# hzi-bifo/RiboDetector

Measured on AMD Instinct MI355X. Metric: reads/sec classified, 100 bp paired-end, higher is better.
Workload: dtype f16x3-split (f32 accumulate); 1 GPU; BASELINE configs[2]: paired-end 100 bp, --ensure rrna, 1048576 pairs/step/GPU x 47 steps (49.3 M total); pinned host bytes -> H2D -> kernels -> labels D2H (SURVEY 8d region ii); read_len=100, ensure=rrna, kernel_variant=mfma_f16x3_t32, parallelism=reads sharded x1, label gather to rank 0, rccl_ranks=1, forced_dist=False, prefix_k=12

## Files before the change

ribodetector_amd/csrc/rd_fastq_index.hpp:

```cpp
#pragma once
#include "rd_common.hpp"

namespace {

constexpr int FQ_THREADS = 256;
constexpr int FQ_BYTES = 64;
constexpr int FQ_TILE = FQ_THREADS * FQ_BYTES;

struct FqSummary {
    int64_t begin, end, n_lines, n_records, consumed;
    unsigned long long bad_record;
    int32_t status, dirty;
    int64_t reserved;
};
static_assert(sizeof(FqSummary) == 64 && sizeof(rd_fq_summary) == 64, "rd_fq_summary layout");

__device__ __forceinline__ bool fq_is_ws(unsigned c) {
    return c == ' ' || (c >= 9 && c <= 13) || (c >= 0x1c && c <= 0x1f) || c == 0x85 || c == 0xa0;
}

__device__ __forceinline__ uint64_t fq_newline_mask(const uint8_t *__restrict__ text, int64_t o, int64_t begin, int64_t end) {
    if (o >= end || o + FQ_BYTES <= begin) return 0;
    const u32x4 *p = reinterpret_cast<const u32x4 *>(text + o);
    uint64_t m = 0;
#pragma unroll
    for (int q = 0; q < 4; ++q) {
        const u32x4 v = p[q];
#pragma unroll
        for (int k = 0; k < 4; ++k) {
            const uint32_t x = v[k] ^ 0x0a0a0a0au;
            const uint32_t z = ~(((x & 0x7f7f7f7fu) + 0x7f7f7f7fu) | x | 0x7f7f7f7fu);
            const uint64_t nib = (((z >> 7) * 0x204081u) >> 21) & 0xfu;
            m |= nib << (16 * q + 4 * k);
        }
    }
    const int lo = begin > o ? (int)(begin - o) : 0, hi = end - o < FQ_BYTES ? (int)(end - o) : FQ_BYTES;
    if (lo > 0) m &= ~0ull << lo;
    if (hi < 64) m &= ~(~0ull << hi);
    return m;
}

__device__ __forceinline__ uint32_t fq_block_scan(uint32_t v, uint32_t *sh, uint32_t &total) {
    const int tid = threadIdx.x, lane = tid & 63, wave = tid >> 6;
    uint32_t inc = v;
#pragma unroll
    for (int o = 1; o < 64; o <<= 1) {
        const uint32_t t = __shfl_up(inc, o);
        if (lane >= o) inc += t;
    }
    if (lane == 63) sh[wave] = inc;
    __syncthreads();
    uint32_t base = 0;
    for (int w = 0; w < wave; ++w) base += sh[w];
    total = sh[0] + sh[1] + sh[2] + sh[3];
    __syncthreads();
    return base + inc - v;
}

template <bool TEXT>
__global__ __launch_bounds__(FQ_THREADS) void rd_fq_begin_kernel(uint8_t *__restrict__ text, int64_t pad, int64_t end, const uint8_t *__restrict__ prev_text,
                                                                const FqSummary *__restrict__ prev, int final, FqSummary *__restrict__ sum) {
    __shared__ int64_t s_begin;
    __shared__ int s_status;
    if (threadIdx.x == 0) {
        int64_t begin = pad;
        int status = RD_FQ_OK;
        if (prev) {
            const int64_t carry = prev->end - prev->consumed;
            if (prev->status != RD_FQ_OK) status = RD_FQ_CHAIN;
            else if (carry < 0 || carry > pad) status = RD_FQ_CARRY;
            else begin = pad - carry;
        }
        s_begin = begin;
        s_status = status;
    }
    __syncthreads();
    const int64_t begin = s_begin;
    if (prev && s_status == RD_FQ_OK) {
        const uint8_t *src = prev_text + prev->consumed;
        for (int64_t i = threadIdx.x; i < pad - begin; i += FQ_THREADS) text[begin + i] = src[i];
    }
    __syncthreads();
    if (threadIdx.x == 0) {
        int64_t e = end;
        if (TEXT && final && e > begin && text[e - 1] != '\n') text[e++] = '\n';
        sum->begin = begin;
        sum->end = e;
        sum->n_lines = sum->n_records = 0;
        sum->consumed = begin;
        sum->bad_record = ~0ull;
        sum->status = s_status;
        sum->dirty = 0;
        sum->reserved = 0;
    }
}

__global__ __launch_bounds__(FQ_THREADS) void rd_fq_count_kernel(const uint8_t *__restrict__ text, const FqSummary *__restrict__ sum,
                                                                uint32_t *__restrict__ tile_count) {
    __shared__ uint32_t sh[4];
    const int64_t o = (int64_t)blockIdx.x * FQ_TILE + (int64_t)threadIdx.x * FQ_BYTES;
    const uint64_t m = sum->status == RD_FQ_OK ? fq_newline_mask(text, o, sum->begin, sum->end) : 0;
    uint32_t total;
    fq_block_scan((uint32_t)__popcll(m), sh, total);
    if (threadIdx.x == 0) tile_count[blockIdx.x] = total;
}

__global__ __launch_bounds__(FQ_THREADS) void rd_fq_scan_kernel(uint32_t *__restrict__ tile_count, int ntiles, FqSummary *__restrict__ sum, int64_t cap_lines) {
    __shared__ uint32_t sh[4];
    __shared__ uint32_t run_s;
    if (threadIdx.x == 0) run_s = 0;
    __syncthreads();
    for (int b0 = 0; b0 < ntiles; b0 += FQ_THREADS) {
        const int b = b0 + threadIdx.x;
        const uint32_t v = b < ntiles ? tile_count[b] : 0;
        uint32_t total;
        const uint32_t ex = fq_block_scan(v, sh, total);
        const uint32_t run = run_s;
        if (b < ntiles) tile_count[b] = run + ex;
        __syncthreads();
        if (threadIdx.x == 0) run_s = run + total;
        __syncthreads();
    }
    if (threadIdx.x == 0) {
        int64_t lines = run_s;
        if (lines > cap_lines) {
            sum->status = RD_FQ_LINES;
            lines = 0;
        }
        sum->n_lines = lines;
        sum->n_records = lines / 4;
    }
}

__global__ __launch_bounds__(FQ_THREADS) void rd_fq_fill_kernel(const uint8_t *__restrict__ text, const FqSummary *__restrict__ sum,
                                                               const uint32_t *__restrict__ tile_base, int32_t *__restrict__ line_end) {
    __shared__ uint32_t sh[4];
    if (sum->status != RD_FQ_OK) return;
    const int64_t o = (int64_t)blockIdx.x * FQ_TILE + (int64_t)threadIdx.x * FQ_BYTES;
    uint64_t m = fq_newline_mask(text, o, sum->begin, sum->end);
    uint32_t total;
    uint32_t j = tile_base[blockIdx.x] + fq_block_scan((uint32_t)__popcll(m), sh, total);
    while (m) {
        const int b = __ffsll((long long)m) - 1;
        line_end[j++] = (int32_t)(o + b);
        m &= m - 1;
    }
}

__device__ __forceinline__ int64_t fq_line_start(const int32_t *__restrict__ line_end, int64_t j, int64_t begin) {
    return j ? (int64_t)line_end[j - 1] + 1 : begin;
}

__global__ __launch_bounds__(FQ_THREADS) void rd_fq_check_kernel(const uint8_t *__restrict__ text, const int32_t *__restrict__ line_end,
                                                                FqSummary *__restrict__ sum, int final) {
    if (sum->status != RD_FQ_OK && sum->status != RD_FQ_TRUNCATED) return;
    const int64_t n = sum->n_records, begin = sum->begin, L = sum->n_lines;
    const int64_t stride = (int64_t)gridDim.x * FQ_THREADS;
    bool dirty = false;
    for (int64_t r = (int64_t)blockIdx.x * FQ_THREADS + threadIdx.x; r < n; r += stride) {
        int64_t ls = fq_line_start(line_end, 4 * r, begin);
        if (text[ls] != '@') atomicMin(&sum->bad_record, (unsigned long long)r);
#pragma unroll
        for (int k = 0; k < 4; ++k) {
            const int64_t p = line_end[4 * r + k];
            dirty |= p > ls && fq_is_ws(text[p - 1]);
            ls = p + 1;
        }
    }
    if (dirty) sum->dirty = 1;
    if (blockIdx.x == 0 && threadIdx.x == 0) {
        int64_t consumed = n ? (int64_t)line_end[4 * n - 1] + 1 : begin;
        if (final) {
            bool trunc = false, ws = false;
            for (int64_t j = 4 * n; j < L; ++j) {
                const int64_t ls = fq_line_start(line_end, j, begin), p = line_end[j];
                if (p > ls) {
                    if (fq_is_ws(text[p - 1])) ws = true; else trunc = true;
                }
            }
            if (ws) sum->dirty = 1;
            else if (trunc) sum->status = RD_FQ_TRUNCATED;
            consumed = sum->end;
        }
        sum->consumed = consumed;
    }
}

__global__ void rd_fq_verdict_kernel(FqSummary *__restrict__ sum) {
    if ((sum->status == RD_FQ_OK || sum->status == RD_FQ_TRUNCATED) && sum->bad_record != ~0ull && !sum->dirty) sum->status = RD_FQ_HEADER;
}

__global__ __launch_bounds__(FQ_THREADS) void rd_fq_gather_kernel(const uint8_t *__restrict__ text, const int32_t *__restrict__ line_end,
                                                                 const FqSummary *__restrict__ sum, int64_t lo, int64_t hi,
                                                                 uint8_t *__restrict__ out_text, int64_t out_cap, const int64_t *__restrict__ cursor_in,
                                                                 int64_t *__restrict__ cursor_out, int64_t *__restrict__ rec_start,
                                                                 int64_t *__restrict__ seq_off, int32_t *__restrict__ seq_len) {
    const int64_t begin = sum->begin;
    const int64_t d0 = *cursor_in;
    const bool framed = sum->status == RD_FQ_OK || sum->status == RD_FQ_HEADER || sum->status == RD_FQ_TRUNCATED;
    const bool ok = framed && hi <= sum->n_records && lo <= hi && d0 >= 0;
    const int64_t src0 = ok ? fq_line_start(line_end, 4 * lo, begin) : 0, src1 = ok ? fq_line_start(line_end, 4 * hi, begin) : 0;
    const int64_t nbytes = src1 - src0;
    const int64_t gtid = (int64_t)blockIdx.x * FQ_THREADS + threadIdx.x, stride = (int64_t)gridDim.x * FQ_THREADS;
    if (!ok || d0 + nbytes > out_cap) {
        if (gtid == 0) *cursor_out = -1;
        return;
    }
    const uint8_t *src = text + src0;
    const int64_t d1 = d0 + nbytes;
    for (int64_t o = (d0 & ~(int64_t)15) + 16 * gtid; o < d1; o += 16 * stride) {
        const int64_t a = o < d0 ? d0 : o, e = o + 16 < d1 ? o + 16 : d1;
        if (a == o && e == o + 16) {
            u32x4 v;
            __builtin_memcpy(&v, src + (o - d0), 16);
            *reinterpret_cast<u32x4 *>(out_text + o) = v;
        } else {
            for (int64_t q = a; q < e; ++q) out_text[q] = src[q - d0];
        }
    }
    const int64_t shift = d0 - src0;
    for (int64_t i = gtid; i < hi - lo; i += stride) {
        const int64_t r = lo + i;
        const int64_t rs = fq_line_start(line_end, 4 * r, begin), so = (int64_t)line_end[4 * r] + 1;
        rec_start[i] = rs + shift;
        seq_off[i] = so + shift;
        seq_len[i] = (int32_t)((int64_t)line_end[4 * r + 1] - so);
    }
    if (gtid == 0) {
        rec_start[hi - lo] = d1;
        *cursor_out = d1;
    }
}

__global__ __launch_bounds__(FQ_THREADS) void rd_fq_strip_mark_kernel(const uint8_t *__restrict__ text, const int32_t *__restrict__ line_end,
                                                                     const FqSummary *__restrict__ sum, uint8_t *__restrict__ del) {
    const int64_t L = sum->n_lines, begin = sum->begin;
    const int64_t stride = (int64_t)gridDim.x * FQ_THREADS;
    for (int64_t j = (int64_t)blockIdx.x * FQ_THREADS + threadIdx.x; j < L; j += stride) {
        const int64_t ls = fq_line_start(line_end, j, begin);
        for (int64_t q = line_end[j]; q > ls && fq_is_ws(text[q - 1]); --q) del[q - 1] = 1;
    }
}

__global__ __launch_bounds__(FQ_THREADS) void rd_fq_sample_kernel(const int32_t *__restrict__ line_end, const FqSummary *__restrict__ sum, int64_t every,
                                                                 int32_t *__restrict__ samples, int64_t cap) {
    const bool framed = sum->status == RD_FQ_OK || sum->status == RD_FQ_HEADER || sum->status == RD_FQ_TRUNCATED;
    const int64_t n = framed ? sum->n_records : -1, begin = sum->begin;
    const int64_t stride = (int64_t)gridDim.x * FQ_THREADS;
    for (int64_t k = (int64_t)blockIdx.x * FQ_THREADS + threadIdx.x; k < cap; k += stride)
        samples[k] = k * every <= n ? (int32_t)fq_line_start(line_end, 4 * k * every, begin) : -1;
}

constexpr int COPY_THREADS = 1024;
__global__ __launch_bounds__(COPY_THREADS) void rd_copy_kernel(uint8_t *__restrict__ dst, const uint8_t *__restrict__ src, int64_t n) {
    const int64_t gtid = (int64_t)blockIdx.x * blockDim.x + threadIdx.x, stride = (int64_t)gridDim.x * blockDim.x;
    const int64_t head = (16 - ((uintptr_t)dst & 15)) & 15;
    if (gtid < head && gtid < n) dst[gtid] = src[gtid];
    const int64_t body = n > head ? (n - head) / 16 : 0;
    u32x4 *d = reinterpret_cast<u32x4 *>(dst + head);
    const uint8_t *s0 = src + head;
    int64_t i = gtid;
    for (; i + 3 * stride < body; i += 4 * stride) {
        u32x4 v0, v1, v2, v3;
        __builtin_memcpy(&v0, s0 + 16 * i, 16);
        __builtin_memcpy(&v1, s0 + 16 * (i + stride), 16);
        __builtin_memcpy(&v2, s0 + 16 * (i + 2 * stride), 16);
        __builtin_memcpy(&v3, s0 + 16 * (i + 3 * stride), 16);
        d[i] = v0; d[i + stride] = v1; d[i + 2 * stride] = v2; d[i + 3 * stride] = v3;
    }
    for (; i < body; i += stride) {
        u32x4 v;
        __builtin_memcpy(&v, s0 + 16 * i, 16);
        d[i] = v;
    }
    const int64_t tail0 = head + 16 * body;
    if (tail0 + gtid < n && gtid < 16) dst[tail0 + gtid] = src[tail0 + gtid];
}

struct FqWs {
    int ntiles;
    uint32_t *tiles;
    size_t total;
};
FqWs fq_ws(Carver &c, int64_t text_end) {
    FqWs p;
    p.ntiles = (int)((text_end + 1 + FQ_TILE - 1) / FQ_TILE);
    if (p.ntiles < 1) p.ntiles = 1;
    p.tiles = c.take<uint32_t>((size_t)p.ntiles);
    p.total = c.off;
    return p;
}
FqWs fq_ws(void *workspace, int64_t text_end) {
    Carver c(workspace);
    return fq_ws(c, text_end);
}

int fq_index_check(const char *fn, const uint8_t *text, int64_t pad, int64_t end, const uint8_t *prev_text, const rd_fq_summary *prev, const int32_t *line_end,
                   int64_t cap_lines, const rd_fq_summary *summary, const void *workspace, bool fa_null, bool fa_bad, const uint8_t *norm) {
    if (!text || !line_end || !summary || !workspace || fa_null) RD_FAIL(RD_E_INVALID, "%s: null pointer", fn);
    if (pad < 0 || end < pad || end >= 0x7fffffffLL - 64 || cap_lines < 0 || fa_bad)
        RD_FAIL(RD_E_INVALID, "%s: bad pad / end / cap_lines%s (a batch buffer is < 2 GiB)", fn, norm ? " / norm_cap / cap_records" : "");
    if ((prev == nullptr) != (prev_text == nullptr)) RD_FAIL(RD_E_INVALID, "%s: prev and prev_text go together", fn);
    if (((uintptr_t)text & 63) || ((uintptr_t)workspace & 255) || ((uintptr_t)norm & 15))
        RD_FAIL(RD_E_INVALID, "%s: text must be 64-byte aligned, workspace 256-byte aligned%s", fn, norm ? ", norm 16-byte aligned" : "");
    return RD_OK;
}

void fq_line_table(uint8_t *text, int64_t pad, int64_t end, const uint8_t *prev_text, const rd_fq_summary *prev, int32_t final, int32_t *line_end, int64_t cap_lines,
                   FqSummary *sum, const FqWs &w, hipStream_t st) {
    hipLaunchKernelGGL(rd_fq_begin_kernel<true>, dim3(1), dim3(FQ_THREADS), 0, st, text, pad, end, prev_text, (const FqSummary *)prev, (int)final, sum);
    hipLaunchKernelGGL(rd_fq_count_kernel, dim3(w.ntiles), dim3(FQ_THREADS), 0, st, text, sum, w.tiles);
    hipLaunchKernelGGL(rd_fq_scan_kernel, dim3(1), dim3(FQ_THREADS), 0, st, w.tiles, w.ntiles, sum, cap_lines);
    hipLaunchKernelGGL(rd_fq_fill_kernel, dim3(w.ntiles), dim3(FQ_THREADS), 0, st, text, sum, w.tiles, line_end);
}

template <typename K, typename... T>
int fq_gather(const char *fn, K kernel, const rd_fq_summary *summary, int64_t rec_lo, int64_t rec_hi, int64_t max_bytes, uint8_t *out_text, int64_t out_cap,
              const int64_t *cursor_in, int64_t *cursor_out, int64_t *rec_start, int64_t *seq_off, int32_t *seq_len, void *stream, T... tables) {
    if ((... || !tables) || !summary || !out_text || !cursor_in || !cursor_out || !rec_start || !seq_off || !seq_len) RD_FAIL(RD_E_INVALID, "%s: null pointer", fn);
    if (rec_lo < 0 || rec_hi < rec_lo || max_bytes < 0 || out_cap < 0 || cursor_in == cursor_out) RD_FAIL(RD_E_INVALID, "%s: bad range", fn);
    if ((uintptr_t)out_text & 15) RD_FAIL(RD_E_INVALID, "%s: out_text must be 16-byte aligned", fn);
    int64_t grid = max_bytes / (16 * FQ_THREADS * 4) + 1;
    const int64_t grid_r = (rec_hi - rec_lo) / FQ_THREADS + 1;
    if (grid < grid_r) grid = grid_r;
    if (grid > 8192) grid = 8192;
    hipLaunchKernelGGL(kernel, dim3((unsigned)grid), dim3(FQ_THREADS), 0, (hipStream_t)stream, tables..., (const FqSummary *)summary, rec_lo, rec_hi, out_text, out_cap,
                       cursor_in, cursor_out, rec_start, seq_off, seq_len);
    RD_HIP(hipGetLastError());
    return RD_OK;
}

template <typename K, typename T>
int fq_sample(const char *fn, K kernel, const T *table, const rd_fq_summary *summary, int64_t every, int32_t *samples, int64_t cap, void *stream) {
    if (!table || !summary || !samples || every < 1 || cap < 0) RD_FAIL(RD_E_INVALID, "%s: bad argument", fn);
    if (cap == 0) return RD_OK;
    int64_t grid = cap / FQ_THREADS + 1;
    if (grid > 1024) grid = 1024;
    hipLaunchKernelGGL(kernel, dim3((unsigned)grid), dim3(FQ_THREADS), 0, (hipStream_t)stream, table, (const FqSummary *)summary, every, samples, cap);
    RD_HIP(hipGetLastError());
    return RD_OK;
}

}
```

ribodetector_amd/csrc/rd_kernels.hip:

```cpp
#include <stdlib.h>
#include "rd_common.hpp"
#include "rd_prep.hpp"
#include "rd_recurrence.hpp"
#include "rd_sort.hpp"
#include "rd_lstm_f32.hpp"
#include "rd_lstm_t32.hpp"
#include "rd_refine.hpp"
#include "rd_encode.hpp"
#include "rd_scan.hpp"
#include "rd_deflate.hpp"
#include "rd_inflate_dev.hpp"
#include "rd_inflate_stream.hpp"
#include "rd_fastq_index.hpp"
#include "rd_fasta_index.hpp"
#include "rd_bam_index.hpp"
#include "rd_bam_shard.hpp"
#include "rd_bam_raw.hpp"
#include "rd_report.hpp"
#include "rd_pairs.hpp"
#include "rd_summary.hpp"
#include "rd_bam_tags.hpp"
#include "rd_bam_tagtext.hpp"
#include "rd_windows.hpp"
#include "rd_regions.hpp"
// ... 613 lines not shown

int rd_gz_inflate_members(const uint8_t *comp, int64_t comp_bytes, const rd_gz_member *members, int64_t n, uint8_t *text, int64_t text_bytes,
                          uint32_t *status, void *stream) {
    static_assert(sizeof(rd_gz_member) == sizeof(GzMemberIn), "rd_gz_member layout");
    if (n < 0 || comp_bytes < 0 || text_bytes < 0) RD_FAIL(RD_E_INVALID, "rd_gz_inflate_members: bad size");
    if (n == 0) return RD_OK;
    if (!comp || !members || !status || (!text && text_bytes > 0)) RD_FAIL(RD_E_INVALID, "rd_gz_inflate_members: null pointer");
    int64_t grid = (n + GZI_WAVES - 1) / GZI_WAVES;
    if (grid > 65536) grid = 65536;
    hipLaunchKernelGGL(rd_gz_inflate_kernel, dim3((unsigned)grid), dim3(64 * GZI_WAVES), 0, (hipStream_t)stream, comp, comp_bytes,
                       (const GzMemberIn *)members, n, text, text_bytes, status);
    RD_HIP(hipGetLastError());
    return RD_OK;
}

namespace {
size_t gzs_workspace_bytes(int64_t data_bytes, int32_t section_bytes, int32_t cap_syms, int64_t text_cap) {
    if (data_bytes < 0 || section_bytes < 1024 || cap_syms < 1024 || text_cap < 0) return 0;
    return gzs_ws(nullptr, data_bytes, section_bytes, cap_syms, text_cap).total;
}

void gzs_crc_fold(const uint8_t *text, int ctiles, GzsState *S, uint32_t *tcrc, hipStream_t st) {
    hipLaunchKernelGGL(rd_gzs_crc_kernel, dim3((unsigned)((ctiles + 3) / 4)), dim3(256), 0, st, text, S, tcrc);
    hipLaunchKernelGGL(rd_gzs_fold_kernel, dim3(1), dim3(64), 0, st, tcrc, S);
}

int gzs_batch(const char *fn, bool range, const uint8_t *comp, int64_t comp_bytes, int64_t data_bytes, int64_t valid_bytes, int32_t section_bytes,
              int32_t cap_syms, uint32_t first_start_bit, const rd_gzs_state *carry, int64_t carry_delta_bits, int32_t at_eof, const void *carried_in,
              void *carried_out, void *text_out, int64_t text_cap, rd_gzs_state *state, void *workspace, size_t workspace_bytes, void *stream) {
    const char *out_name = range ? "sym_text" : "text";
    const unsigned out_align = range ? 16 : 8;
    if (!comp || !carried_out || !text_out || !state || !workspace) RD_FAIL(RD_E_INVALID, "%s: null pointer", fn);
    if (((uintptr_t)comp & 3) || ((uintptr_t)workspace & 255) || ((uintptr_t)text_out & (out_align - 1)))
        RD_FAIL(RD_E_INVALID, "%s: comp must be 4-byte aligned, %s %u-byte aligned, workspace 256-byte aligned", fn, out_name, out_align);
    if (data_bytes <= 0 || valid_bytes < data_bytes || comp_bytes < valid_bytes || valid_bytes >= (1LL << 28) || section_bytes < 1024 || (section_bytes & 3) ||
        cap_syms < 1024 || text_cap < 0)
        RD_FAIL(RD_E_INVALID, "%s: bad sizes (a batch holds < 256 MiB of compressed bytes)", fn);
    if (range && (carry == nullptr) != (carried_in == nullptr))
        RD_FAIL(RD_E_INVALID, "%s: carry and map_in go together (both null: the range's first batch)", fn);
    const GzsWs p = gzs_ws(workspace, data_bytes, section_bytes, cap_syms, text_cap);
    if (workspace_bytes < p.total) RD_FAIL(RD_E_WORKSPACE, "%s: workspace too small: %zu < %zu", fn, workspace_bytes, p.total);
    hipStream_t st = (hipStream_t)stream;
    const uint32_t end_bits = (uint32_t)(valid_bytes * 8), sec_bits = (uint32_t)section_bytes * 8u;
    GzsState *S = (GzsState *)state;
    const GzsState *C = (const GzsState *)carry;
    const int search0 = (range && C == nullptr && first_start_bit == GZS_SEARCH) ? 1 : 0;
    const dim3 resolve_grid((unsigned)(p.nsec * p.tiles_per_sec));
    hipLaunchKernelGGL(rd_gzs_search_kernel, dim3((unsigned)((p.nsec + 1 + GZS_WAVES - 1) / GZS_WAVES)), dim3(64 * GZS_WAVES), 0, st, comp, comp_bytes, end_bits, sec_bits,
                       p.nsec, first_start_bit, C, carry_delta_bits, p.found);
    hipLaunchKernelGGL(rd_gzs_decode_kernel, dim3((unsigned)((p.nsec + GZS_WAVES - 1) / GZS_WAVES)), dim3(64 * GZS_WAVES), 0, st, comp, comp_bytes, end_bits, p.nsec, p.found,
                       p.syms, (int)cap_syms, p.sec);
    hipLaunchKernelGGL(rd_gzs_scan_kernel, dim3(1), dim3(64), 0, st, p.sec, p.found, p.nsec, (int)at_eof, text_cap, p.off, p.wslot, p.plist, S, C, search0);
    hipLaunchKernelGGL(rd_gzs_symwin_kernel, dim3((unsigned)p.ngroups), dim3(1024), 0, st, p.syms, (int)cap_syms, p.sec, p.plist, p.wslot, p.nsec, S, p.windows16, p.gmaps);
    if (!range) {
        hipLaunchKernelGGL(rd_gzs_chain_kernel, dim3(1), dim3(1024), 0, st, p.gmaps, p.wslot, p.nsec, S, (const uint8_t *)carried_in, (const uint16_t *)nullptr, 1, p.gwin,
                           (uint16_t *)nullptr, (uint8_t *)carried_out);
        hipLaunchKernelGGL(rd_gzs_resolve_kernel<false>, resolve_grid, dim3(256), 0, st, p.syms, (int)cap_syms, p.sec, p.found, p.off, p.wslot, p.tiles_per_sec, p.windows16,
                           p.gwin, S, (uint8_t *)text_out, (uint16_t *)nullptr);
        gzs_crc_fold((const uint8_t *)text_out, p.ctiles, S, p.tcrc, st);
    } else {
        hipLaunchKernelGGL(rd_gzs_chain_kernel, dim3(1), dim3(1024), 0, st, p.gmaps, p.wslot, p.nsec, S, (const uint8_t *)nullptr, (const uint16_t *)carried_in, 0, p.gwin,
                           (uint16_t *)carried_out, (uint8_t *)nullptr);
        hipLaunchKernelGGL(rd_gzs_resolve_kernel<true>, resolve_grid, dim3(256), 0, st, p.syms, (int)cap_syms, p.sec, p.found, p.off, p.wslot, p.tiles_per_sec, p.windows16,
                           p.gwin, S, (uint8_t *)nullptr, (uint16_t *)text_out);
    }
    RD_HIP(hipGetLastError());
    return RD_OK;
}
}

size_t rd_gz_stream_workspace_bytes(int64_t data_bytes, int32_t section_bytes, int32_t cap_syms, int64_t text_cap) {
    return gzs_workspace_bytes(data_bytes, section_bytes, cap_syms, text_cap);
}

int rd_gz_stream_inflate(const uint8_t *comp, int64_t comp_bytes, int64_t data_bytes, int64_t valid_bytes, int32_t section_bytes, int32_t cap_syms,
                         uint32_t first_start_bit, const rd_gzs_state *carry, int64_t carry_delta_bits, int32_t at_eof, const uint8_t *win_in,
                         uint8_t *win_out, uint8_t *text, int64_t text_cap, rd_gzs_state *state, void *workspace, size_t workspace_bytes, void *stream) {
    return gzs_batch("rd_gz_stream_inflate", false, comp, comp_bytes, data_bytes, valid_bytes, section_bytes, cap_syms, first_start_bit, carry, carry_delta_bits,
                     at_eof, win_in, win_out, text, text_cap, state, workspace, workspace_bytes, stream);
}

size_t rd_gz_range_workspace_bytes(int64_t data_bytes, int32_t section_bytes, int32_t cap_syms, int64_t text_cap) {
    return gzs_workspace_bytes(data_bytes, section_bytes, cap_syms, text_cap);
}

int rd_gz_range_decode(const uint8_t *comp, int64_t comp_bytes, int64_t data_bytes, int64_t valid_bytes, int32_t section_bytes, int32_t cap_syms,
                       uint32_t first_start_bit, const rd_gzs_state *carry, int64_t carry_delta_bits, int32_t at_eof, const uint16_t *map_in, uint16_t *map_out,
                       uint16_t *sym_text, int64_t text_cap, rd_gzs_state *state, void *workspace, size_t workspace_bytes, void *stream) {
    return gzs_batch("rd_gz_range_decode", true, comp, comp_bytes, data_bytes, valid_bytes, section_bytes, cap_syms, first_start_bit, carry, carry_delta_bits,
                     at_eof, map_in, map_out, sym_text, text_cap, state, workspace, workspace_bytes, stream);
}

size_t rd_gz_range_resolve_workspace_bytes(int64_t n) { return n < 0 ? 0 : ((size_t)(n / GZS_CTILE + 2) * 4 + 255) / 256 * 256; }

int rd_gz_range_resolve(const uint16_t *sym_text, int64_t n, const uint8_t *window, uint32_t win_valid, uint8_t *text, rd_gzs_state *state, void *workspace,
                        size_t workspace_bytes, void *stream) {
    if (n < 0 || !state || (n > 0 && (!sym_text || !text || !workspace))) RD_FAIL(RD_E_INVALID, "rd_gz_range_resolve: bad argument");
    if (win_valid > 0 && !window) RD_FAIL(RD_E_INVALID, "rd_gz_range_resolve: win_valid > 0 needs a window");
    if (((uintptr_t)sym_text & 15) || ((uintptr_t)text & 15)) RD_FAIL(RD_E_INVALID, "rd_gz_range_resolve: sym_text and text must be 16-byte aligned");
    if (workspace_bytes < rd_gz_range_resolve_workspace_bytes(n)) RD_FAIL(RD_E_WORKSPACE, "rd_gz_range_resolve: workspace too small");
    hipStream_t st = (hipStream_t)stream;
    GzsState *S = (GzsState *)state;
    int64_t grid = n / (8 * 256 * 4) + 1;
    if (grid > 4096) grid = 4096;
    hipLaunchKernelGGL(rd_gzs_symtext_kernel, dim3((unsigned)grid), dim3(256), 0, st, sym_text, n, window, win_valid, text, S);
    gzs_crc_fold(text, (int)((n + GZS_CTILE - 1) / GZS_CTILE) + 1, S, (uint32_t *)workspace, st);
    RD_HIP(hipGetLastError());
    return RD_OK;
}

int rd_stream_create(int device, const uint32_t *cu_mask, int words, int priority, void **stream) {
    if (!stream || words < 0 || (words > 0 && !cu_mask)) RD_FAIL(RD_E_INVALID, "rd_stream_create: bad argument");
    RD_HIP(hipSetDevice(device));
    hipStream_t st = nullptr;
    if (words > 0) {
        RD_HIP(hipExtStreamCreateWithCUMask(&st, (uint32_t)words, cu_mask));
    } else {
        int lo = 0, hi = 0;
        RD_HIP(hipDeviceGetStreamPriorityRange(&lo, &hi));
        RD_HIP(hipStreamCreateWithPriority(&st, hipStreamNonBlocking, priority < 0 ? hi : lo));
    }
    *stream = (void *)st;
    return RD_OK;
}

int rd_stream_destroy(void *stream) {
    if (stream) RD_HIP(hipStreamDestroy((hipStream_t)stream));
    return RD_OK;
}

int rd_copy_bytes(void *dst, const void *src, int64_t n, int32_t workgroups, void *stream) {
    if (n < 0 || (n > 0 && (!dst || !src))) RD_FAIL(RD_E_INVALID, "rd_copy_bytes: bad argument");
    if (n == 0) return RD_OK;
    int64_t grid = workgroups > 0 ? workgroups : 8;
    const int64_t need = n / (16 * COPY_THREADS) + 1;
    if (grid > need) grid = need;
    hipLaunchKernelGGL(rd_copy_kernel, dim3((unsigned)grid), dim3(COPY_THREADS), 0, (hipStream_t)stream, (uint8_t *)dst, (const uint8_t *)src, n);
    RD_HIP(hipGetLastError());
    return RD_OK;
}

size_t rd_fastq_index_workspace_bytes(int64_t text_end) {
    if (text_end < 0 || text_end >= 0x7fffffffLL) return 0;
    return fq_ws(nullptr, text_end).total;
}

int rd_fastq_index(uint8_t *text, int64_t pad, int64_t end, const uint8_t *prev_text, const rd_fq_summary *prev, int32_t final, int32_t *line_end,
                   int64_t cap_lines, rd_fq_summary *summary, void *workspace, size_t workspace_bytes, void *stream) {
    if (const int rc = fq_index_check("rd_fastq_index", text, pad, end, prev_text, prev, line_end, cap_lines, summary, workspace, false, false, nullptr)) return rc;
    const FqWs p = fq_ws(workspace, end);
    if (workspace_bytes < p.total) RD_FAIL(RD_E_WORKSPACE, "rd_fastq_index: workspace too small: %zu < %zu", workspace_bytes, p.total);
    hipStream_t st = (hipStream_t)stream;
    FqSummary *sum = (FqSummary *)summary;
    fq_line_table(text, pad, end, prev_text, prev, final, line_end, cap_lines, sum, p, st);
    int grid = (int)((end - pad) / (64 * FQ_THREADS)) + 1;
    if (grid > 2048) grid = 2048;
    hipLaunchKernelGGL(rd_fq_check_kernel, dim3(grid), dim3(FQ_THREADS), 0, st, text, line_end, sum, (int)final);
    hipLaunchKernelGGL(rd_fq_verdict_kernel, dim3(1), dim3(1), 0, st, sum);
    RD_HIP(hipGetLastError());
    return RD_OK;
}

int rd_fastq_gather(const uint8_t *text, const int32_t *line_end, const rd_fq_summary *summary, int64_t rec_lo, int64_t rec_hi, int64_t max_bytes,
                    uint8_t *out_text, int64_t out_cap, const int64_t *cursor_in, int64_t *cursor_out, int64_t *rec_start, int64_t *seq_off,
                    int32_t *seq_len, void *stream) {
    return fq_gather("rd_fastq_gather", rd_fq_gather_kernel, summary, rec_lo, rec_hi, max_bytes, out_text, out_cap, cursor_in, cursor_out, rec_start, seq_off, seq_len,
                     stream, text, line_end);
}

int rd_fastq_sample(const int32_t *line_end, const rd_fq_summary *summary, int64_t every, int32_t *samples, int64_t cap, void *stream) {
    return fq_sample("rd_fastq_sample", rd_fq_sample_kernel, line_end, summary, every, samples, cap, stream);
}

int rd_fastq_strip_mark(const uint8_t *text, const int32_t *line_end, const rd_fq_summary *summary, int64_t max_lines, uint8_t *del, void *stream) {
    if (!text || !line_end || !summary || !del || max_lines < 0) RD_FAIL(RD_E_INVALID, "rd_fastq_strip_mark: bad argument");
    int64_t grid = max_lines / FQ_THREADS + 1;
    if (grid > 4096) grid = 4096;
    hipLaunchKernelGGL(rd_fq_strip_mark_kernel, dim3((unsigned)grid), dim3(FQ_THREADS), 0, (hipStream_t)stream, text, line_end, (const FqSummary *)summary, del);
    RD_HIP(hipGetLastError());
    return RD_OK;
}

size_t rd_fasta_index_workspace_bytes(int64_t text_end, int64_t cap_lines) {
    if (text_end < 0 || text_end >= 0x7fffffffLL || cap_lines < 0) return 0;
    return fa_ws(nullptr, text_end, cap_lines).total;
}

int rd_fasta_index(uint8_t *text, int64_t pad, int64_t end, const uint8_t *prev_text, const rd_fq_summary *prev, int32_t final, int32_t *line_end,
                   int64_t cap_lines, uint8_t *norm, int64_t norm_cap, int64_t *rec_tab, int32_t *hdr_tab, int64_t cap_records, rd_fq_summary *summary,
                   void *workspace, size_t workspace_bytes, void *stream) {
    if (const int rc = fq_index_check("rd_fasta_index", text, pad, end, prev_text, prev, line_end, cap_lines, summary, workspace, !norm || !rec_tab || !hdr_tab,
                                      norm_cap < 0 || cap_records < 1, norm))
        return rc;
    const FaWs p = fa_ws(workspace, end, cap_lines);
    if (workspace_bytes < p.total) RD_FAIL(RD_E_WORKSPACE, "rd_fasta_index: workspace too small: %zu < %zu", workspace_bytes, p.total);
    hipStream_t st = (hipStream_t)stream;
    FqSummary *sum = (FqSummary *)summary;
    fq_line_table(text, pad, end, prev_text, prev, final, line_end, cap_lines, sum, p.fq, st);
    hipLaunchKernelGGL(rd_fa_init_kernel, dim3(1), dim3(FQ_THREADS), 0, st, p.sc);
    hipLaunchKernelGGL(rd_fa_lines_kernel, dim3(p.nblk), dim3(FQ_THREADS), 0, st, text, line_end, sum, p.info_a, p.info_k, p.blk, p.sc);
    hipLaunchKernelGGL(rd_fa_base_kernel, dim3(1), dim3(FQ_THREADS), 0, st, p.blk, line_end, sum, p.sc, (int)final, norm_cap, cap_records, norm, rec_tab, hdr_tab);
    hipLaunchKernelGGL(rd_fa_emit_kernel, dim3(p.nblk), dim3(FQ_THREADS), 0, st, text, p.info_a, p.info_k, p.blk, sum, p.sc, (int)final, norm, rec_tab, hdr_tab);
    RD_HIP(hipGetLastError());
    return RD_OK;
}

int rd_fasta_gather(const uint8_t *norm, const int64_t *rec_tab, const int32_t *hdr_tab, const rd_fq_summary *summary, int64_t rec_lo, int64_t rec_hi,
                    int64_t max_bytes, uint8_t *out_text, int64_t out_cap, const int64_t *cursor_in, int64_t *cursor_out, int64_t *rec_start,
                    int64_t *seq_off, int32_t *seq_len, void *stream) {
    return fq_gather("rd_fasta_gather", rd_fa_gather_kernel<false>, summary, rec_lo, rec_hi, max_bytes, out_text, out_cap, cursor_in, cursor_out, rec_start, seq_off, seq_len,
                     stream, norm, rec_tab, hdr_tab);
}

int rd_fasta_sample(const int64_t *rec_tab, const rd_fq_summary *summary, int64_t every, int32_t *samples, int64_t cap, void *stream) {
    return fq_sample("rd_fasta_sample", rd_fa_sample_kernel<false>, rec_tab, summary, every, samples, cap, stream);
}

size_t rd_bam_index_workspace_bytes(int64_t text_end) {
    if (text_end < 0 || text_end >= 0x7fffffffLL) return 0;
    return bam_ws(nullptr, text_end).total;
}

int rd_bam_index(uint8_t *text, int64_t pad, int64_t end, const uint8_t *prev_text, const rd_fq_summary *prev, int32_t final, uint8_t *norm, int64_t norm_cap,
                 int64_t *rec_tab, int32_t *hdr_tab, int64_t cap_records, rd_fq_summary *summary, void *workspace, size_t workspace_bytes, void *stream) {
    if (const int rc = fq_index_check("rd_bam_index", text, pad, end, prev_text, prev, (const int32_t *)text, 0, summary, workspace, !norm || !rec_tab || !hdr_tab,
                                      norm_cap < 0 || cap_records < 1, norm))
        return rc;
    const BamWs p = bam_ws(workspace, end);
    if (workspace_bytes < p.total) RD_FAIL(RD_E_WORKSPACE, "rd_bam_index: workspace too small: %zu < %zu", workspace_bytes, p.total);
    hipStream_t st = (hipStream_t)stream;
    FqSummary *sum = (FqSummary *)summary;
    hipLaunchKernelGGL(rd_fq_begin_kernel<false>, dim3(1), dim3(FQ_THREADS), 0, st, text, pad, end, prev_text, (const FqSummary *)prev, (int)final, sum);
    hipLaunchKernelGGL(rd_bam_walk_kernel<true>, dim3(p.nseg), dim3(64), 0, st, text, sum, p.seg, p.lists);
    hipLaunchKernelGGL(rd_bam_stitch_kernel<true>, dim3(1), dim3(64), 0, st, text, sum, p.seg, p.lists, p.nseg, p.seg_rbase, p.seg_nbase, p.seg_cnt, p.sc, (int)final, norm_cap,
                       cap_records, rec_tab);
    hipLaunchKernelGGL(rd_bam_table_kernel, dim3(p.nseg), dim3(64), 0, st, text, sum, p.sc, p.lists, p.seg_rbase, p.seg_nbase, p.seg_cnt, rec_tab, hdr_tab, p.src_tab);
    int64_t grid = (4 * end / 3 + 64) / BAM_EMIT_BYTES + 1;
    if (grid > 65536) grid = 65536;
    hipLaunchKernelGGL(rd_bam_emit_kernel, dim3((unsigned)grid), dim3(FQ_THREADS), 0, st, text, sum, rec_tab, p.src_tab, norm, norm_cap);
    RD_HIP(hipGetLastError());
    return RD_OK;
}

int rd_bam_gather(const uint8_t *norm, const int64_t *rec_tab, const int32_t *hdr_tab, const rd_fq_summary *summary, int64_t rec_lo, int64_t rec_hi,
                  int64_t max_bytes, uint8_t *out_text, int64_t out_cap, const int64_t *cursor_in, int64_t *cursor_out, int64_t *rec_start,
                  int64_t *seq_off, int32_t *seq_len, void *stream) {
    return fq_gather("rd_bam_gather", rd_fa_gather_kernel<true>, summary, rec_lo, rec_hi, max_bytes, out_text, out_cap, cursor_in, cursor_out, rec_start, seq_off, seq_len,
                     stream, norm, rec_tab, hdr_tab);
}

int rd_bam_sample(const int64_t *rec_tab, const rd_fq_summary *summary, int64_t every, int32_t *samples, int64_t cap, void *stream) {
    return fq_sample("rd_bam_sample", rd_fa_sample_kernel<true>, rec_tab, summary, every, samples, cap, stream);
}

int rd_bam_find_start(const uint8_t *text, int64_t lo, int64_t hi, int64_t end, int32_t at_eof, int64_t *info, void *stream) {
    if (!info || (!text && end > 0)) RD_FAIL(RD_E_INVALID, "rd_bam_find_start: null pointer");
    if ((uintptr_t)text & 15) RD_FAIL(RD_E_INVALID, "rd_bam_find_start: text must be 16-byte aligned");
    hipStream_t st = (hipStream_t)stream;
    const bool bad = lo < 0 || hi < lo || end < hi || end >= 0x7fffffffLL;
    hipLaunchKernelGGL(rd_bam_find_init_kernel, dim3(1), dim3(1), 0, st, (unsigned long long *)info, bad ? 1 : 0);
    if (!bad && hi > lo) {
        const int64_t grid = (hi - lo + BAM_FIND_CAND - 1) / BAM_FIND_CAND;
        hipLaunchKernelGGL(rd_bam_find_kernel, dim3((unsigned)grid), dim3(BAM_FIND_THREADS), 0, st, text, lo, hi, end, (int)at_eof, (unsigned long long *)info);
    }
    RD_HIP(hipGetLastError());
    return RD_OK;
}

size_t rd_bam_count_workspace_bytes(int64_t text_end) {
    if (text_end < 0 || text_end >= 0x7fffffffLL) return 0;
    return bam_count_ws(nullptr, text_end).total;
}

int rd_bam_count(uint8_t *text, int64_t pad, int64_t end, const uint8_t *prev_text, const rd_fq_summary *prev, int32_t final, rd_fq_summary *summary, void *workspace,
                 size_t workspace_bytes, void *stream) {
    if (const int rc = fq_index_check("rd_bam_count", text, pad, end, prev_text, prev, (const int32_t *)text, 0, summary, workspace, false, false, nullptr)) return rc;
    const BamCountWs p = bam_count_ws(workspace, end);
    if (workspace_bytes < p.total) RD_FAIL(RD_E_WORKSPACE, "rd_bam_count: workspace too small: %zu < %zu", workspace_bytes, p.total);
    hipStream_t st = (hipStream_t)stream;
    FqSummary *sum = (FqSummary *)summary;
    hipLaunchKernelGGL(rd_fq_begin_kernel<false>, dim3(1), dim3(FQ_THREADS), 0, st, text, pad, end, prev_text, (const FqSummary *)prev, (int)final, sum);
    hipLaunchKernelGGL(rd_bam_walk_kernel<false>, dim3(p.nseg), dim3(64), 0, st, text, sum, p.seg, (int2 *)nullptr);
    hipLaunchKernelGGL(rd_bam_stitch_kernel<false>, dim3(1), dim3(64), 0, st, text, sum, p.seg, (int2 *)nullptr, p.nseg, (int32_t *)nullptr, (int64_t *)nullptr,
                       (int32_t *)nullptr, (BamScratch *)nullptr, (int)final, (int64_t)0, (int64_t)0, (int64_t *)nullptr);
    RD_HIP(hipGetLastError());
    return RD_OK;
}

int32_t *rd_bam_index_src(void *workspace, int64_t text_end) {
    if (!workspace || text_end < 0 || text_end >= 0x7fffffffLL) return nullptr;
    return bam_ws(workspace, text_end).src_tab;
}

int rd_bam_raw_tab(const uint8_t *text, const int32_t *src_tab, const rd_fq_summary *summary, int64_t *raw_tab, int64_t cap_records, int64_t every, int32_t *samples,
                   int64_t cap_samples, void *stream) {
    if (!text || !src_tab || !summary || !raw_tab || (cap_samples > 0 && !samples)) RD_FAIL(RD_E_INVALID, "rd_bam_raw_tab: null pointer");
    if (cap_records < 1 || cap_records > 0x7fffffffLL || every < 1 || cap_samples < 0) RD_FAIL(RD_E_INVALID, "rd_bam_raw_tab: bad cap_records / every / cap_samples");
    hipStream_t st = (hipStream_t)stream;
    const FqSummary *sum = (const FqSummary *)summary;
    const unsigned nb = (unsigned)((cap_records + GZ_SCAN_ITEMS - 1) / GZ_SCAN_ITEMS);
    hipLaunchKernelGGL(rd_bam_raw_local_kernel, dim3(nb), dim3(256), 0, st, text, src_tab, sum, raw_tab, cap_records);
    hipLaunchKernelGGL(rd_bam_raw_base_kernel, dim3(1), dim3(256), 0, st, sum, raw_tab);
    hipLaunchKernelGGL(rd_bam_raw_add_kernel, dim3(nb), dim3(256), 0, st, sum, raw_tab);
    if (cap_samples > 0) {
        int64_t grid = cap_samples / FQ_THREADS + 1;
        if (grid > 1024) grid = 1024;
        hipLaunchKernelGGL(rd_bam_raw_sample_kernel, dim3((unsigned)grid), dim3(FQ_THREADS), 0, st, (const int64_t *)raw_tab, sum, every, samples, cap_samples);
    }
    RD_HIP(hipGetLastError());
    return RD_OK;
}

int rd_bam_raw_gather(const uint8_t *text, const int32_t *src_tab, const int64_t *raw_tab, const rd_fq_summary *summary, int64_t rec_lo, int64_t rec_hi,
                      int64_t max_bytes, uint8_t *out, int64_t out_cap, const int64_t *cursor_in, int64_t *cursor_out, int64_t *raw_start, void *stream) {
    if (!text || !src_tab || !raw_tab || !summary || !out || !cursor_in || !cursor_out || !raw_start) RD_FAIL(RD_E_INVALID, "rd_bam_raw_gather: null pointer");
    if (rec_lo < 0 || rec_hi < rec_lo || max_bytes < 0 || out_cap < 0 || cursor_in == cursor_out) RD_FAIL(RD_E_INVALID, "rd_bam_raw_gather: bad range");
    if ((uintptr_t)out & 15) RD_FAIL(RD_E_INVALID, "rd_bam_raw_gather: out must be 16-byte aligned");
    int64_t grid = max_bytes / (BAM_RAW_BYTES * 4) + 1;
    const int64_t grid_r = (rec_hi - rec_lo) / FQ_THREADS + 1;
    if (grid < grid_r) grid = grid_r;
    if (grid > 8192) grid = 8192;
    hipLaunchKernelGGL(rd_bam_raw_gather_kernel, dim3((unsigned)grid), dim3(FQ_THREADS), 0, (hipStream_t)stream, text, src_tab, raw_tab, (const FqSummary *)summary, rec_lo,
                       rec_hi, out, out_cap, cursor_in, cursor_out, raw_start);
    RD_HIP(hipGetLastError());
    return RD_OK;
}

namespace {
struct ReportWs {
    int nb;
    int32_t *idlen, *fault;
    uint64_t *qs;
    int64_t *bsum;
    size_t total;
};
ReportWs report_ws(void *workspace, int64_t n) {
    ReportWs p;
    Carver c(workspace);
    p.nb = scan_blocks(n);
    p.idlen = c.take<int32_t>((size_t)n);
    p.qs = c.take<uint64_t>((size_t)n);
    p.bsum = c.take<int64_t>((size_t)p.nb);
    p.fault = c.take<int32_t>(1);
    p.total = c.off;
    return p;
}
}

size_t rd_report_workspace_bytes(int64_t n) {
    if (n < 0) return 0;
    return report_ws(nullptr, n).total;
// ... 405 lines not shown
```

Measured before the change: 35.31 million reads/s.

## Fuse FASTQ record validation into line-fill kernel and parallelize tile scan

```diff
diff --git a/ribodetector_amd/csrc/rd_fastq_index.hpp b/ribodetector_amd/csrc/rd_fastq_index.hpp
--- a/ribodetector_amd/csrc/rd_fastq_index.hpp
+++ b/ribodetector_amd/csrc/rd_fastq_index.hpp
@@ -107,22 +107,18 @@
 
 __global__ __launch_bounds__(FQ_THREADS) void rd_fq_scan_kernel(uint32_t *__restrict__ tile_count, int ntiles, FqSummary *__restrict__ sum, int64_t cap_lines) {
     __shared__ uint32_t sh[4];
-    __shared__ uint32_t run_s;
-    if (threadIdx.x == 0) run_s = 0;
-    __syncthreads();
-    for (int b0 = 0; b0 < ntiles; b0 += FQ_THREADS) {
-        const int b = b0 + threadIdx.x;
-        const uint32_t v = b < ntiles ? tile_count[b] : 0;
-        uint32_t total;
-        const uint32_t ex = fq_block_scan(v, sh, total);
-        const uint32_t run = run_s;
-        if (b < ntiles) tile_count[b] = run + ex;
-        __syncthreads();
-        if (threadIdx.x == 0) run_s = run + total;
-        __syncthreads();
+    const int per = (ntiles + FQ_THREADS - 1) / FQ_THREADS;
+    const int b0 = (int)threadIdx.x * per < ntiles ? (int)threadIdx.x * per : ntiles, b1 = b0 + per < ntiles ? b0 + per : ntiles;
+    uint32_t s = 0, total;
+    for (int b = b0; b < b1; ++b) s += tile_count[b];
+    uint32_t run = fq_block_scan(s, sh, total);
+    for (int b = b0; b < b1; ++b) {
+        const uint32_t v = tile_count[b];
+        tile_count[b] = run;
+        run += v;
     }
     if (threadIdx.x == 0) {
-        int64_t lines = run_s;
+        int64_t lines = total;
         if (lines > cap_lines) {
             sum->status = RD_FQ_LINES;
             lines = 0;
@@ -132,62 +128,66 @@
     }
 }
 
-__global__ __launch_bounds__(FQ_THREADS) void rd_fq_fill_kernel(const uint8_t *__restrict__ text, const FqSummary *__restrict__ sum,
-                                                               const uint32_t *__restrict__ tile_base, int32_t *__restrict__ line_end) {
+__device__ __forceinline__ int64_t fq_line_start(const int32_t *__restrict__ line_end, int64_t j, int64_t begin) {
+    return j ? (int64_t)line_end[j - 1] + 1 : begin;
+}
+
+template <bool CHECK>
+__global__ __launch_bounds__(FQ_THREADS) void rd_fq_fill_kernel(const uint8_t *__restrict__ text, FqSummary *sum, const uint32_t *__restrict__ tile_base,
+                                                               int32_t *__restrict__ line_end) {
     __shared__ uint32_t sh[4];
     if (sum->status != RD_FQ_OK) return;
+    const int64_t begin = sum->begin, end = sum->end, L = sum->n_lines;
     const int64_t o = (int64_t)blockIdx.x * FQ_TILE + (int64_t)threadIdx.x * FQ_BYTES;
-    uint64_t m = fq_newline_mask(text, o, sum->begin, sum->end);
+    uint64_t m = fq_newline_mask(text, o, begin, end);
+    uint64_t ws = 0, no_at = 0;
+    if (CHECK) {
+        for (uint64_t q = m; q; q &= q - 1) {
+            const int b = __ffsll((long long)q) - 1;
+            const int64_t p = o + b;
+            const unsigned c = p > begin ? text[p - 1] : '\n';
+            if (c != '\n' && fq_is_ws(c)) ws |= 1ull << b;
+            if (p + 1 < end && text[p + 1] != '@') no_at |= 1ull << b;
+        }
+    }
     uint32_t total;
-    uint32_t j = tile_base[blockIdx.x] + fq_block_scan((uint32_t)__popcll(m), sh, total);
+    int64_t j = tile_base[blockIdx.x] + fq_block_scan((uint32_t)__popcll(m), sh, total);
+    const int64_t in_records = L & ~(int64_t)3;
+    bool dirty = false;
     while (m) {
         const int b = __ffsll((long long)m) - 1;
-        line_end[j++] = (int32_t)(o + b);
+        line_end[j] = (int32_t)(o + b);
+        if (CHECK && j < in_records) {
+            dirty |= (ws >> b) & 1;
+            if ((j & 3) == 3 && j + 1 < in_records && ((no_at >> b) & 1)) atomicMin(&sum->bad_record, (unsigned long long)((j + 1) >> 2));
+        }
+        ++j;
         m &= m - 1;
     }
-}
-
-__device__ __forceinline__ int64_t fq_line_start(const int32_t *__restrict__ line_end, int64_t j, int64_t begin) {
-    return j ? (int64_t)line_end[j - 1] + 1 : begin;
-}
-
-__global__ __launch_bounds__(FQ_THREADS) void rd_fq_check_kernel(const uint8_t *__restrict__ text, const int32_t *__restrict__ line_end,
-                                                                FqSummary *__restrict__ sum, int final) {
-    if (sum->status != RD_FQ_OK && sum->status != RD_FQ_TRUNCATED) return;
+    if (CHECK && dirty) sum->dirty = 1;
+}
+
+__global__ void rd_fq_verdict_kernel(const uint8_t *__restrict__ text, const int32_t *__restrict__ line_end, FqSummary *__restrict__ sum, int final) {
+    if (sum->status != RD_FQ_OK) return;
     const int64_t n = sum->n_records, begin = sum->begin, L = sum->n_lines;
-    const int64_t stride = (int64_t)gridDim.x * FQ_THREADS;
-    bool dirty = false;
-    for (int64_t r = (int64_t)blockIdx.x * FQ_THREADS + threadIdx.x; r < n; r += stride) {
-        int64_t ls = fq_line_start(line_end, 4 * r, begin);
-        if (text[ls] != '@') atomicMin(&sum->bad_record, (unsigned long long)r);
-#pragma unroll
-        for (int k = 0; k < 4; ++k) {
-            const int64_t p = line_end[4 * r + k];
-            dirty |= p > ls && fq_is_ws(text[p - 1]);
-            ls = p + 1;
-        }
-    }
-    if (dirty) sum->dirty = 1;
-    if (blockIdx.x == 0 && threadIdx.x == 0) {
-        int64_t consumed = n ? (int64_t)line_end[4 * n - 1] + 1 : begin;
-        if (final) {
-            bool trunc = false, ws = false;
-            for (int64_t j = 4 * n; j < L; ++j) {
-                const int64_t ls = fq_line_start(line_end, j, begin), p = line_end[j];
-                if (p > ls) {
-                    if (fq_is_ws(text[p - 1])) ws = true; else trunc = true;
-                }
+    if (n && text[begin] != '@') sum->bad_record = 0;
+    int64_t consumed = n ? (int64_t)line_end[4 * n - 1] + 1 : begin;
+    int status = RD_FQ_OK, dirty = sum->dirty;
+    if (final) {
+        bool trunc = false, ws = false;
+        for (int64_t j = 4 * n; j < L; ++j) {
+            const int64_t ls = fq_line_start(line_end, j, begin), p = line_end[j];
+            if (p > ls) {
+                if (fq_is_ws(text[p - 1])) ws = true; else trunc = true;
             }
-            if (ws) sum->dirty = 1;
-            else if (trunc) sum->status = RD_FQ_TRUNCATED;
-            consumed = sum->end;
-        }
-        sum->consumed = consumed;
-    }
-}
-
-__global__ void rd_fq_verdict_kernel(FqSummary *__restrict__ sum) {
-    if ((sum->status == RD_FQ_OK || sum->status == RD_FQ_TRUNCATED) && sum->bad_record != ~0ull && !sum->dirty) sum->status = RD_FQ_HEADER;
+        }
+        if (ws) sum->dirty = dirty = 1;
+        else if (trunc) status = RD_FQ_TRUNCATED;
+        consumed = sum->end;
+    }
+    sum->consumed = consumed;
+    if (sum->bad_record != ~0ull && !dirty) status = RD_FQ_HEADER;
+    if (status != RD_FQ_OK) sum->status = status;
 }
 
 __global__ __launch_bounds__(FQ_THREADS) void rd_fq_gather_kernel(const uint8_t *__restrict__ text, const int32_t *__restrict__ line_end,
@@ -306,12 +306,14 @@
     return RD_OK;
 }
 
+template <bool CHECK>
 void fq_line_table(uint8_t *text, int64_t pad, int64_t end, const uint8_t *prev_text, const rd_fq_summary *prev, int32_t final, int32_t *line_end, int64_t cap_lines,
                    FqSummary *sum, const FqWs &w, hipStream_t st) {
     hipLaunchKernelGGL(rd_fq_begin_kernel<true>, dim3(1), dim3(FQ_THREADS), 0, st, text, pad, end, prev_text, (const FqSummary *)prev, (int)final, sum);
     hipLaunchKernelGGL(rd_fq_count_kernel, dim3(w.ntiles), dim3(FQ_THREADS), 0, st, text, sum, w.tiles);
     hipLaunchKernelGGL(rd_fq_scan_kernel, dim3(1), dim3(FQ_THREADS), 0, st, w.tiles, w.ntiles, sum, cap_lines);
-    hipLaunchKernelGGL(rd_fq_fill_kernel, dim3(w.ntiles), dim3(FQ_THREADS), 0, st, text, sum, w.tiles, line_end);
+    hipLaunchKernelGGL(rd_fq_fill_kernel<CHECK>, dim3(w.ntiles), dim3(FQ_THREADS), 0, st, text, sum, w.tiles, line_end);
+    if (CHECK) hipLaunchKernelGGL(rd_fq_verdict_kernel, dim3(1), dim3(1), 0, st, text, line_end, sum, (int)final);
 }
 
 template <typename K, typename... T>
diff --git a/ribodetector_amd/csrc/rd_kernels.hip b/ribodetector_amd/csrc/rd_kernels.hip
--- a/ribodetector_amd/csrc/rd_kernels.hip
+++ b/ribodetector_amd/csrc/rd_kernels.hip
@@ -789,11 +789,7 @@
     if (workspace_bytes < p.total) RD_FAIL(RD_E_WORKSPACE, "rd_fastq_index: workspace too small: %zu < %zu", workspace_bytes, p.total);
     hipStream_t st = (hipStream_t)stream;
     FqSummary *sum = (FqSummary *)summary;
-    fq_line_table(text, pad, end, prev_text, prev, final, line_end, cap_lines, sum, p, st);
-    int grid = (int)((end - pad) / (64 * FQ_THREADS)) + 1;
-    if (grid > 2048) grid = 2048;
-    hipLaunchKernelGGL(rd_fq_check_kernel, dim3(grid), dim3(FQ_THREADS), 0, st, text, line_end, sum, (int)final);
-    hipLaunchKernelGGL(rd_fq_verdict_kernel, dim3(1), dim3(1), 0, st, sum);
+    fq_line_table<true>(text, pad, end, prev_text, prev, final, line_end, cap_lines, sum, p, st);
     RD_HIP(hipGetLastError());
     return RD_OK;
 }
@@ -833,7 +829,7 @@
     if (workspace_bytes < p.total) RD_FAIL(RD_E_WORKSPACE, "rd_fasta_index: workspace too small: %zu < %zu", workspace_bytes, p.total);
     hipStream_t st = (hipStream_t)stream;
     FqSummary *sum = (FqSummary *)summary;
-    fq_line_table(text, pad, end, prev_text, prev, final, line_end, cap_lines, sum, p.fq, st);
+    fq_line_table<false>(text, pad, end, prev_text, prev, final, line_end, cap_lines, sum, p.fq, st);
     hipLaunchKernelGGL(rd_fa_init_kernel, dim3(1), dim3(FQ_THREADS), 0, st, p.sc);
     hipLaunchKernelGGL(rd_fa_lines_kernel, dim3(p.nblk), dim3(FQ_THREADS), 0, st, text, line_end, sum, p.info_a, p.info_k, p.blk, p.sc);
     hipLaunchKernelGGL(rd_fa_base_kernel, dim3(1), dim3(FQ_THREADS), 0, st, p.blk, line_end, sum, p.sc, (int)final, norm_cap, cap_records, norm, rec_tab, hdr_tab);
```

After: 35.22 million reads/s. No clear change (-0.2%).
